# ootts/EasyHeC

Hardware: AMD Instinct MI355X
Metric: mask-render fwd+bwd frames/sec, xArm7 50k-tri @1280x720x8-view (higher is better)
Workload: dtype f32; 1 GPU; xarm7_1280x720_8view; robot=xarm7 (41096 tris, 20525 verts), views_per_gpu=8, global_views=8, links=8, antialias=True, optimizer=Adam lr 3e-3 wd 5e-4, ref_sums=bound once, mask_output=False, step=HIP launch chain, parallelism=single GPU

## Files before the change

easyhec_amd/csrc/ehr_fused_core.h:

```cpp
#pragma once
#include "ehr_host.h"
#include "ehr_pose_core.h"
#include "ehr_raster_core.h"

namespace ehr {

#define EHR_FIX_SCALE 4294967296.0
__device__ __forceinline__ long long fix_of(float v) { return __double2ll_rn((double)v * EHR_FIX_SCALE); }
__device__ __forceinline__ void fix_add(long long* acc, float v, int* meta) {
    if (!(fabsf(v) < 1.0e9f)) {
        atomicOr(&meta[EHR_META_OVERFLOW], 1);
        return;
    }
    if (v != 0.f) atomicAdd((unsigned long long*)acc, (unsigned long long)fix_of(v));
}
__device__ __forceinline__ void fix_add_delta(long long* acc, float v, long long cached, int* meta) {
    if (!(fabsf(v) < 1.0e9f)) {
        atomicOr(&meta[EHR_META_OVERFLOW], 1);
        return;
    }
    const long long d = ((v != 0.f) ? fix_of(v) : 0ll) - cached;
    if (d != 0) atomicAdd((unsigned long long*)acc, (unsigned long long)d);
}
__device__ __forceinline__ float fix_get(long long q) { return (float)((double)q * (1.0 / EHR_FIX_SCALE)); }
__device__ __forceinline__ long long acc_load(const long long* p) {
    return __hip_atomic_load(p, __ATOMIC_RELAXED, __HIP_MEMORY_SCOPE_AGENT);
}

__host__ __device__ constexpr int vb_acc_stride(int L, int nls = VB_LOSS_SLOTS) { return 12 * L + nls * VB_LOSS_STRIDE; }
__host__ __device__ __forceinline__ int* vb_acc_meta(long long* acc, int B, int L) { return (int*)(acc + (size_t)B * vb_acc_stride(L)); }

struct StepTail {
    const float* K;
    const float* link_poses;
    const float* tc_jac;
    float* red;
    float* dof;
    float* m;
    float* v;
    int* step;
    float* loss_out;
    float* grad_out;
    float n, f, lr, b1, b2, eps, wd;
    int defer_adam;
};

template <bool TAIL>
__device__ __forceinline__ void finish_body(const BinGeom& g, int B, const long long* __restrict__ facc,
                                            const long long* __restrict__ vtot, float* __restrict__ loss,
                                            float* __restrict__ grad_mvp, int* __restrict__ meta, const StepTail& tail,
                                            int nls, int* __restrict__ lbox, int lstride, float* vloss ,
                                            double (*S)[17] , float* red_lds ,
                                            float (*Js)[16] ) {
    const int tid = threadIdx.x, L = g.L;
    const int acc_stride = vb_acc_stride(L, nls);
    if (lbox)
        for (int i = tid; i < 16 * B * L; i += 256) lbox[i] = (i & 2) ? INT_MIN : INT_MAX;
    AdamState st;
    if (TAIL && !tail.defer_adam) st = pose_adam_fetch(tail.dof, tail.m, tail.v, tail.step);
    auto view_loss_slow = [&](int b) {
        long long s = vtot ? vtot[b] : 0ll;
        for (int k = 0; k < nls; k++) s += acc_load(&facc[(size_t)b * acc_stride + 12 * L + k * lstride]);
        return fix_get(s);
    };
    const bool bad = __hip_atomic_load(&meta[EHR_META_OVERFLOW], __ATOMIC_RELAXED, __HIP_MEMORY_SCOPE_AGENT) != 0;
    const float nanv = __int_as_float(0x7fc00000);
    double la_mine = 0.0;
    if (nls == 32) {
        const int k = tid & 31;
        for (int base = 0; base < B; base += 32) {
            long long s4[4];
#pragma unroll
            for (int j = 0; j < 4; j++) {
                const int b = base + 8 * j + (tid >> 5);
                s4[j] = (b < B) ? acc_load(&facc[(size_t)b * acc_stride + 12 * L + k * lstride]) : 0;
            }
            if (TAIL && base == 0 && !tail.defer_adam) pose_adam_bias(st, tail.lr, tail.b1, tail.b2);
#pragma unroll
            for (int j = 0; j < 4; j++) {
                const int b = base + 8 * j + (tid >> 5);
                if (base + 8 * j >= B) break;
                long long s = s4[j];
                s += wave_xor<16>(s);
                s += wave_xor<8>(s);
                s += wave_xor<4>(s);
                s += wave_xor<2>(s);
                s += wave_xor<1>(s);
                if (k == 0 && b < B) {
                    const float lv = bad ? nanv : fix_get(s + (vtot ? vtot[b] : 0ll));
                    loss[b] = lv;
                    la_mine += (double)lv;
                }
            }
        }
    } else {
        for (int b = tid; b < B; b += 256) {
            const float lv = bad ? nanv : view_loss_slow(b);
            loss[b] = lv;
            la_mine += (double)lv;
        }
    }
    auto grad16 = [&](int bl, float* G) {
        const int b = bl / L, l = bl - b * L;
        const long long* a = facc + (size_t)b * acc_stride + 12 * l;
        long long q[12];
#pragma unroll
        for (int e = 0; e < 12; e++) q[e] = acc_load(a + e);
#pragma unroll
        for (int e = 0; e < 16; e++) {
            const int r = e >> 2, c = e & 3;
            float v = 0.f;
            if (r != 2) v = fix_get(q[4 * (r == 3 ? 2 : r) + c]);
            G[e] = bad ? nanv : v;
        }
    };
    if (!TAIL) {
        if (grad_mvp)
            for (int i = tid; i < B * L; i += 256) {
                float G[16];
                grad16(i, G);
#pragma unroll
                for (int e = 0; e < 16; e++) grad_mvp[(size_t)i * 16 + e] = G[e];
            }
        return;
    }
    pose_backward_block_t(
        [&](int i, float* G) {
            grad16(i, G);
            if (grad_mvp)
#pragma unroll
                for (int e = 0; e < 16; e++) grad_mvp[(size_t)i * 16 + e] = G[e];
        },
        [&](int) { return 0.f; }, tail.K, tail.link_poses, tail.tc_jac, B, L, g.H, g.W, tail.n, tail.f, tail.red, S, red_lds,
        &la_mine, nls == 32, Js);
    __syncthreads();
    if (!tail.defer_adam)
        pose_adam_apply(st, tail.dof, tail.m, tail.v, tail.step, red_lds, tail.lr, tail.b1, tail.b2, tail.eps, tail.wd,
                        tail.loss_out, tail.grad_out);
}


static inline BinGeom make_geom(int H, int W, int L) {
    BinGeom g;
    g.W = W;
    g.H = H;
    g.ntx = (W + EHR_TILE_W - 1) / EHR_TILE_W;
    g.nty = (H + EHR_TILE_H - 1) / EHR_TILE_H;
    g.nt = g.ntx * g.nty;
    g.L = L;
    return g;
}

struct StepHead {
    const float* dof;
    const float* K;
    const float* link_poses;
    float* tc_jac;
    int* hist_row;
    float* history;
    int history_rows;
    float n, f;
    const int* adam_step;
    int* hstate;
};


}
```

easyhec_amd/csrc/ehr_pose_core.h:

```cpp
#pragma once
#include "ehr_device.h"

namespace ehr {

template <int N>
struct Dual {
    float v;
    float d[N];
};
template <int N>
__device__ __forceinline__ Dual<N> dconst(float c) {
    Dual<N> r;
    r.v = c;
#pragma unroll
    for (int i = 0; i < N; i++) r.d[i] = 0.f;
    return r;
}
template <int N>
__device__ __forceinline__ Dual<N> operator+(const Dual<N>& a, const Dual<N>& b) {
    Dual<N> r;
    r.v = a.v + b.v;
#pragma unroll
    for (int i = 0; i < N; i++) r.d[i] = a.d[i] + b.d[i];
    return r;
}
template <int N>
__device__ __forceinline__ Dual<N> operator-(const Dual<N>& a, const Dual<N>& b) {
    Dual<N> r;
    r.v = a.v - b.v;
#pragma unroll
    for (int i = 0; i < N; i++) r.d[i] = a.d[i] - b.d[i];
    return r;
}
template <int N>
__device__ __forceinline__ Dual<N> operator*(const Dual<N>& a, const Dual<N>& b) {
    Dual<N> r;
    r.v = a.v * b.v;
#pragma unroll
    for (int i = 0; i < N; i++) r.d[i] = a.d[i] * b.v + a.v * b.d[i];
    return r;
}
template <int N>
__device__ __forceinline__ Dual<N> operator/(const Dual<N>& a, const Dual<N>& b) {
    Dual<N> r;
    float inv = 1.f / b.v;
    r.v = a.v * inv;
#pragma unroll
    for (int i = 0; i < N; i++) r.d[i] = (a.d[i] - r.v * b.d[i]) * inv;
    return r;
}
template <int N>
__device__ __forceinline__ Dual<N> dneg(const Dual<N>& a) {
    return dconst<N>(0.f) - a;
}
template <int N>
__device__ __forceinline__ Dual<N> dsqrt(const Dual<N>& a) {
    Dual<N> r;
    r.v = sqrtf(a.v);
    float k = 0.5f / r.v;
#pragma unroll
    for (int i = 0; i < N; i++) r.d[i] = a.d[i] * k;
    return r;
}
template <int N>
__device__ __forceinline__ Dual<N> dsin(const Dual<N>& a) {
    Dual<N> r;
    r.v = sinf(a.v);
    float c = cosf(a.v);
#pragma unroll
    for (int i = 0; i < N; i++) r.d[i] = a.d[i] * c;
    return r;
}
template <int N>
__device__ __forceinline__ Dual<N> dcos(const Dual<N>& a) {
    Dual<N> r;
    r.v = cosf(a.v);
    float s = -sinf(a.v);
#pragma unroll
    for (int i = 0; i < N; i++) r.d[i] = a.d[i] * s;
    return r;
}
template <int N>
__device__ __forceinline__ Dual<N> dclamp_min(const Dual<N>& a, float eps) {
    return (a.v >= eps) ? a : dconst<N>(eps);
}

typedef Dual<6> D6;

template <int N>
__device__ void se3_exp_dual(const float* dof, float eps, Dual<N> T[16], int which = 0) {
    Dual<N> x[6];
#pragma unroll
    for (int i = 0; i < 6; i++) {
        x[i] = dconst<N>(dof[i]);
        if (N == 6) x[i].d[i % N] = 1.f;
        else if (i == which) x[i].d[0] = 1.f;
    }
    const Dual<N> u0 = x[0], u1 = x[1], u2 = x[2], w0 = x[3], w1 = x[4], w2 = x[5];
    Dual<N> nrms = w0 * w0 + w1 * w1 + w2 * w2;
    Dual<N> th = dsqrt(dclamp_min(nrms, eps));
    Dual<N> one = dconst<N>(1.f), zero = dconst<N>(0.f);
    Dual<N> inv = one / th;
    Dual<N> fac1 = inv * dsin(th);
    Dual<N> fac2 = inv * inv * (one - dcos(th));
    Dual<N> K[9] = {zero, dneg(w2), w1, w2, zero, dneg(w0), dneg(w1), w0, zero};
    Dual<N> K2[9];
    for (int r = 0; r < 3; r++)
        for (int c = 0; c < 3; c++) K2[3 * r + c] = K[3 * r] * K[c] + K[3 * r + 1] * K[3 + c] + K[3 * r + 2] * K[6 + c];
    Dual<N> fv1 = (one - dcos(th)) / (th * th);
    Dual<N> fv2 = (th - dsin(th)) / (th * th * th);
    Dual<N> u[3] = {u0, u1, u2};
    for (int r = 0; r < 3; r++) {
        Dual<N> t = zero;
        for (int c = 0; c < 3; c++) {
            Dual<N> I = dconst<N>(r == c ? 1.f : 0.f);
            T[4 * r + c] = fac1 * K[3 * r + c] + fac2 * K2[3 * r + c] + I;
            Dual<N> V = I + K[3 * r + c] * fv1 + K2[3 * r + c] * fv2;
            t = t + V * u[c];
        }
        T[4 * r + 3] = t;
    }
    T[12] = zero;
    T[13] = zero;
    T[14] = zero;
    T[15] = one;
}

__device__ __forceinline__ void mat4_mul(const float* A, const float* B, float* C) {
    for (int r = 0; r < 4; r++)
        for (int c = 0; c < 4; c++) {
            float s = A[4 * r] * B[c];
            s = fmaf(A[4 * r + 1], B[4 + c], s);
            s = fmaf(A[4 * r + 2], B[8 + c], s);
            s = fmaf(A[4 * r + 3], B[12 + c], s);
            C[4 * r + c] = s;
        }
}

__device__ __forceinline__ void projection(const float* K, int H, int W, float n, float f, float* P) {
    float fu = K[0], fv = K[4], cu = K[2], cv = K[5];
    for (int i = 0; i < 16; i++) P[i] = 0.f;
    P[0] = 2.f * fu / (float)W;
    P[2] = -2.f * cu / (float)W + 1.f;
    P[5] = 2.f * fv / (float)H;
    P[6] = 2.f * cv / (float)H - 1.f;
    P[10] = -(f + n) / (f - n);
    P[11] = -2.f * f * n / (f - n);
    P[14] = -1.f;
}


__device__ __forceinline__ void mvp_from_pose(const float* Tc, const float* P, const float* lp, float* C) {
    float A[16];
    mat4_mul(Tc, lp, A);
    for (int c = 0; c < 4; c++) {
        A[4 + c] = -A[4 + c];
        A[8 + c] = -A[8 + c];
    }
    mat4_mul(P, A, C);
}

__device__ __forceinline__ double wave_sum_f64(double v) {
    v += wave_xor<32>(v);
    v += wave_xor<16>(v);
    v += wave_xor<8>(v);
    v += wave_xor<4>(v);
    v += wave_xor<2>(v);
    v += wave_xor<1>(v);
    return v;
}
template <class GetG, class GetLoss>
__device__ __forceinline__ void pose_backward_block_t(GetG get_g, GetLoss get_loss, const float* __restrict__ K,
                                                      const float* __restrict__ link_poses,
                                                      const float* __restrict__ tc_jac, int B, int L, int H, int W,
                                                      float n, float f, float* __restrict__ red, double (*S)[17],
                                                      float* red_lds, const double* la_pre,
                                                      bool la_lanes_0_32, float (*Js_lds)[16]) {
    float (*const Js)[16] = Js_lds;
    if (threadIdx.x < 96) Js[threadIdx.x >> 4][threadIdx.x & 15] = tc_jac[16 + threadIdx.x];
    float P[16];
    projection(K, H, W, n, f, P);
    for (int r = 0; r < 4; r++) {
        P[4 * r + 1] = -P[4 * r + 1];
        P[4 * r + 2] = -P[4 * r + 2];
    }
    const int r = threadIdx.x & 3;
    double acc[4] = {0.0, 0.0, 0.0, 0.0};
    double la = 0.0;
    for (int i = threadIdx.x >> 2; i < B * L; i += blockDim.x >> 2) {
        float lp[16];
#pragma unroll
        for (int k = 0; k < 16; k++) lp[k] = link_poses[(size_t)i * 16 + k];
        float G[16];
        get_g(i, G);
        float M[4];
        for (int c = 0; c < 4; c++) {
            float s = 0.f;
            for (int k = 0; k < 4; k++) s = fmaf(P[4 * k + r], G[4 * k + c], s);
            M[c] = s;
        }
        for (int c = 0; c < 4; c++) {
            float s = 0.f;
            for (int k = 0; k < 4; k++) s = fmaf(M[k], lp[4 * c + k], s);
            acc[c] += (double)s;
        }
    }
    if (la_pre)
        la = *la_pre;
    else
        for (int i = threadIdx.x; i < B; i += blockDim.x) la += (double)get_loss(i);
    const int lane = threadIdx.x & 63, wave = threadIdx.x >> 6;
    {
        const bool b32 = lane & 32, b16 = lane & 16;
        const double a0 = (b32 ? acc[2] : acc[0]) + wave_xor<32>(b32 ? acc[0] : acc[2]);
        const double a1 = (b32 ? acc[3] : acc[1]) + wave_xor<32>(b32 ? acc[1] : acc[3]);
        double v = (b16 ? a1 : a0) + wave_xor<16>(b16 ? a0 : a1);
        v += wave_xor<8>(v);
        v += wave_xor<4>(v);
        if ((lane & 12) == 0) S[wave][4 * (lane & 3) + 2 * (b32 ? 1 : 0) + (b16 ? 1 : 0)] = v;
    }
    {
        const double s = la_lanes_0_32 ? la + wave_xor<32>(la) : wave_sum_f64(la);
        if (lane == 0) S[wave][16] = s;
    }
    __syncthreads();
    if (threadIdx.x < 8) {
        float rr;
        if (threadIdx.x < 6) {
            double g = 0.0;
            for (int k = 0; k < 16; k++)
                g += (((S[0][k] + S[1][k]) + S[2][k]) + S[3][k]) * (double)Js[threadIdx.x][k];
            rr = (float)g;
        } else {
            rr = (threadIdx.x == 6) ? (float)(((S[0][16] + S[1][16]) + S[2][16]) + S[3][16]) : (float)B;
        }
        red[threadIdx.x] = rr;
        if (red_lds) red_lds[threadIdx.x] = rr;
    }
}

__device__ __forceinline__ void pose_backward_block(const float* __restrict__ grad_mvp, const float* __restrict__ loss,
                                                    const float* __restrict__ K, const float* __restrict__ link_poses,
                                                    const float* __restrict__ tc_jac, int B, int L, int H, int W,
                                                    float n, float f, float* __restrict__ red, double (*S)[17]) {
    __shared__ float Js[6][16];
    pose_backward_block_t(
        [&](int i, float* G) {
            for (int k = 0; k < 16; k++) G[k] = grad_mvp[(size_t)i * 16 + k];
        },
        [&](int b) { return loss[b]; }, K, link_poses, tc_jac, B, L, H, W, n, f, red, S, nullptr, nullptr, false, Js);
}

struct AdamState {
    float p, m, v;
    int t;
    float step_size, rsq_bc2;
    bool has_bias;
};
__device__ __forceinline__ void pose_adam_bias(AdamState& st, float lr, float b1, float b2) {
    const float bc1 = 1.f - powf(b1, (float)st.t);
    const float bc2 = 1.f - powf(b2, (float)st.t);
    st.step_size = lr / bc1;
    st.rsq_bc2 = sqrtf(bc2);
    st.has_bias = true;
}
__device__ __forceinline__ AdamState pose_adam_fetch(const float* dof, const float* m, const float* v, const int* step) {
    AdamState st;
    st.p = st.m = st.v = 0.f;
    st.step_size = st.rsq_bc2 = 0.f;
    st.has_bias = false;
    st.t = step[0] + 1;
    if (threadIdx.x < 6) {
        st.p = dof[threadIdx.x];
        st.m = m[threadIdx.x];
        st.v = v[threadIdx.x];
    }
    return st;
}
__device__ __forceinline__ void pose_adam_apply(const AdamState& st, float* __restrict__ dof, float* __restrict__ m,
                                                float* __restrict__ v, int* __restrict__ step, const float* red, float lr,
                                                float b1, float b2, float eps, float wd, float* __restrict__ loss_out,
                                                float* __restrict__ grad_out) {
    const int i = threadIdx.x;
    const int t = st.t;
    const float nfr = red[7];
    bool ok = true;
#pragma unroll
    for (int k = 0; k < 8; k++) ok = ok && (fabsf(red[k]) < 3.0e38f);
    if (i < 6 && ok) {
        float g = red[i] / nfr;
        if (grad_out) grad_out[i] = g;
        float p = st.p;
        g = g + wd * p;
        float mi = b1 * st.m + (1.f - b1) * g;
        float vi = b2 * st.v + (1.f - b2) * g * g;
        m[i] = mi;
        v[i] = vi;
        float step_size, rsq_bc2;
        if (st.has_bias) {
            step_size = st.step_size;
            rsq_bc2 = st.rsq_bc2;
        } else {
            const float bc1 = 1.f - powf(b1, (float)t);
            const float bc2 = 1.f - powf(b2, (float)t);
            step_size = lr / bc1;
            rsq_bc2 = sqrtf(bc2);
        }
        float denom = sqrtf(vi) / rsq_bc2 + eps;
        dof[i] = p - step_size * (mi / denom);
    }
    if (i < 6 && !ok && grad_out) grad_out[i] = __int_as_float(0x7fc00000);
    if (i == 6 && loss_out) loss_out[0] = ok ? red[6] / nfr : __int_as_float(0x7fc00000);
    __syncthreads();
    if (i == 0 && ok) step[0] = t;
}
__device__ __forceinline__ void pose_adam_block(float* __restrict__ dof, float* __restrict__ m, float* __restrict__ v,
                                                int* __restrict__ step, const float* __restrict__ red, float lr,
                                                float b1, float b2, float eps, float wd, float* __restrict__ loss_out,
                                                float* __restrict__ grad_out) {
    const AdamState st = pose_adam_fetch(dof, m, v, step);
    pose_adam_apply(st, dof, m, v, step, red, lr, b1, b2, eps, wd, loss_out, grad_out);
}

}
```

easyhec_amd/csrc/ehr_vbuf.hip:

```cpp
#include <stdlib.h>
#include <string.h>

#include <algorithm>
#include <utility>
#include <vector>

#include "ehr_fused_core.h"

namespace ehr {

constexpr int VB_RW = EHR_TILE_W + 2;
constexpr int VB_RH = EHR_TILE_H + 2;
constexpr int VB_RN = VB_RW * VB_RH;
constexpr int VB_WORDS = (VB_RN + 63) / 64;
constexpr int VB_LBOX_STRIDE = 16;
constexpr int VB_HEAVY_T_DEFAULT = 3000;
constexpr int VB_HEAVY_CAP = 4096;
constexpr int VB_MED_CAP = 2048;
constexpr int VB_MED_T_DEFAULT = 1500;
constexpr int VB_PRIO_LONG = 3;
constexpr int VB_PRIO_HEAVY = 2;
constexpr int VB_JOB_ITEMS = 64;
constexpr int VB_SPILL_BLOCK = 2048;
constexpr u64 VB_EMPTY = ~0ull;
constexpr int VB_VERTEX_GRID = 5;
constexpr int VB_JOB_GRID = 4;
constexpr int VB_COMPOSITE_GRID = 6;
constexpr int VB_SCORE_COUNT_GRID = 4;
constexpr int VB_SLOW_GRID = 32;
constexpr bool VB_XCD_SPLIT = true;
constexpr int VB_FAST_EXTENT = 8192;

constexpr int VB_XCDS = 8;
constexpr int VB_XCD_BITS = __builtin_ctz(VB_XCDS);
static_assert(VB_XCDS == 1 << VB_XCD_BITS, "a workgroup finds its XCD with a mask and a shift");
__host__ __device__ constexpr int vb_xcd_share(int n) { return (n + VB_XCDS - 1) >> VB_XCD_BITS; }
__host__ __device__ constexpr int vb_xcd_round_up(int n) { return (n + VB_XCDS - 1) & ~(VB_XCDS - 1); }

enum VbLine {
    VB_LINE_JOB_CURSOR = 0,
    VB_LINE_COMP_TICKET = VB_LINE_JOB_CURSOR + VB_XCDS,
    VB_LINE_TOP_TICKET = VB_LINE_COMP_TICKET + VB_XCDS,
    VB_LINE_SLOW_COUNT,
    VB_LINES
};
__host__ __device__ __forceinline__ int* vb_line(int* meta, int k) {
    return (int*)((((uintptr_t)(meta + EHR_META_INTS)) + 127) & ~(uintptr_t)127) + 32 * k;
}
constexpr size_t VB_META_BYTES = EHR_META_INTS * sizeof(int) + (VB_LINES + 1) * 128;

#define VB_WAVE_SYNC() asm volatile("s_waitcnt lgkmcnt(0)" ::: "memory")

struct VbItem {
    int packed;
    int v1, v2;
    float alpha;
};

struct VbCarve {
    uintptr_t at;
    template <class T>
    T* take(size_t n, size_t align = alignof(T)) {
        at = (at + align - 1) & ~(uintptr_t)(align - 1);
        T* const p = (T*)at;
        at += n * sizeof(T);
        return p;
    }
};

struct VbSlots {
    float* jval;
    VbItem* jitems;
    u64* jcov;
    int* jn;
    int* jspill;
    unsigned* jid;
    int* jdesc;
    int* jbase;
    unsigned* jutile;
    int4* slow_list;
    int jcap;
};
constexpr size_t VB_SLOT_BYTES = 256 * sizeof(float) + VB_JOB_ITEMS * sizeof(VbItem) + VB_WORDS * sizeof(u64) + 2 * sizeof(int) +
                                 VB_RN * sizeof(unsigned) + sizeof(int) + sizeof(int4);
static_assert(VB_SLOT_BYTES == 1024 + 1024 + 48 + 8 + 1360 + 4 + 16, "job slot: 3484 bytes");
static VbSlots vb_slots(void* base, size_t jcap, size_t units, size_t* bytes = nullptr) {
    VbCarve c{(uintptr_t)base};
    VbSlots s;
    s.jval = c.take<float>(jcap * 256);
    s.jitems = c.take<VbItem>(jcap * VB_JOB_ITEMS);
    s.jcov = c.take<u64>(jcap * VB_WORDS);
    s.jn = c.take<int>(jcap);
    s.jspill = c.take<int>(jcap);
    s.jid = c.take<unsigned>(jcap * VB_RN);
    s.jdesc = c.take<int>(jcap);
    s.jbase = c.take<int>(units + 1);
    s.jutile = c.take<unsigned>(units);
    s.slow_list = c.take<int4>(jcap, 16);
    s.jcap = (int)jcap;
    if (bytes) *bytes = c.at - (uintptr_t)base;
    return s;
}

constexpr bool vb_interior(int i) {
    return (i % VB_RW) >= 1 && (i % VB_RW) <= EHR_TILE_W && (i / VB_RW) >= 1 && (i / VB_RW) <= EHR_TILE_H;
}
constexpr u64 vb_word_h(int k) {
    u64 w = 0;
    for (int j = 0; j < 64; j++) {
        const int i = 64 * k + j;
        if (i + 1 < VB_RN && (i % VB_RW) != VB_RW - 1 && (vb_interior(i) || vb_interior(i + 1))) w |= 1ull << j;
    }
    return w;
}
constexpr u64 vb_word_v(int k) {
    u64 w = 0;
    for (int j = 0; j < 64; j++) {
        const int i = 64 * k + j;
        if (i + VB_RW < VB_RN && (vb_interior(i) || vb_interior(i + VB_RW))) w |= 1ull << j;
    }
    return w;
}

template <int S>
__device__ __forceinline__ void vb_shr(const u64 in[VB_WORDS], u64 out[VB_WORDS]) {
#pragma unroll
    for (int k = 0; k < VB_WORDS; k++) out[k] = (in[k] >> S) | (k + 1 < VB_WORDS ? in[k + 1] << (64 - S) : 0ull);
}

__device__ __forceinline__ int vb_readlane(int v, int lane) { return __builtin_amdgcn_readlane(v, lane); }
__device__ __forceinline__ float vb_readlane(float v, int lane) {
    return __int_as_float(__builtin_amdgcn_readlane(__float_as_int(v), lane));
}
__device__ __forceinline__ float4 vb_readlane(const float4& v, int lane) {
    return make_float4(vb_readlane(v.x, lane), vb_readlane(v.y, lane), vb_readlane(v.z, lane), vb_readlane(v.w, lane));
}
__device__ __forceinline__ int vb_mbcnt(u64 m) {
    return __builtin_amdgcn_mbcnt_hi((unsigned)(m >> 32), __builtin_amdgcn_mbcnt_lo((unsigned)m, 0u));
}


struct VbHeavy {
    int* gen;
    int* list;
    int* mlist;
    int* stamp;
    int mcap;
    int heavy_base;
    int heavy_max;
};

static VbHeavy vb_heavy(void* base, size_t nstamp, size_t* bytes = nullptr) {
    VbCarve c{(uintptr_t)base};
    VbHeavy hv = {};
    hv.gen = c.take<int>(8);
    hv.list = c.take<int>(2 * VB_HEAVY_CAP);
    hv.mlist = c.take<int>(2 * VB_MED_CAP);
    hv.stamp = c.take<int>(nstamp);
    if (bytes) *bytes = c.at - (uintptr_t)base;
    return hv;
}

__device__ __forceinline__ int vb_hint_pack(int u, int tx, int ty) { return tx | (ty << 10) | (u << 22); }
__device__ __forceinline__ int vb_hint_dense(int id, int nt, int ntx) {
    return (int)((unsigned)id >> 22) * nt + ((id >> 10) & 4095) * ntx + (id & 1023);
}
static_assert(VB_MAX_UNITS <= 1024, "vb_hint_pack");
struct VbClusters {
    const int32_t* ctri;
    const int32_t* clink;
    const int32_t* coff;
    const float* laabb;
    const float4* cvert;
    int NC;
};

__device__ __forceinline__ uint2 vb_pack_box(int x0, int y0, int x1, int y1) {
    return make_uint2((unsigned)x0 | ((unsigned)y0 << 16), (unsigned)x1 | ((unsigned)y1 << 16));
}
#define VB_BOX_EMPTY make_uint2(0xffffffffu, 0u)

struct VbEdges {
    int e0, e1, e2, sx0, sx1, sx2, sy0, sy1, sy2;
};
__device__ __forceinline__ VbEdges vb_edges(int X0, int Y0, int X1, int Y1, int X2, int Y2, int bx0, int by0, int W,
                                            int H) {
    VbEdges r;
    const int ox = 16 * bx0 + 8 - 8 * W, oy = 16 * by0 + 8 - 8 * H;
    X0 -= ox; X1 -= ox; X2 -= ox;
    Y0 -= oy; Y1 -= oy; Y2 -= oy;
    {
        const int dX = X1 - X0, dY = Y1 - Y0;
        r.e0 = __mul24(dX, 0 - Y0) - __mul24(dY, 0 - X0) - (((dY < 0) || (dY == 0 && dX < 0)) ? 0 : 1);
        r.sx0 = -16 * dY;
        r.sy0 = 16 * dX;
    }
// ... 1849 lines not shown
        if (lane < VB_RH) S.cov[lane] = 0ull;
        if (COVER && lane == 0) S.bad = 0;
        VB_WAVE_SYNC();
        int nsurv = 0, dln = 0;
        const int drawn = vb_job_raster<false, COVER, LAZY>(A, S, S.key, S.cov, b, l, rg, rx0, ry0, 0, 1, nsurv, dln);
        if (COVER) {
            if (drawn >= 0 && dln > 0)
                vb_flush<true, LAZY>(S, S.key, S.cov, dln, VbLazy{pverts, pmvp + ((size_t)b * L + l) * 16, LAZY ? nullptr : posc + (size_t)b * V}, PRM(si.cvidx) + (size_t)lcoff[l] * 64, W, H, rx0, ry0);
            VB_WAVE_SYNC();
            if (drawn < 0 || S.bad) {
                if (lane == 0) PRM(rq.sl.jn)[0] = 1;
                continue;
            }
            if (drawn > 0) {
                VB_WAVE_SYNC();
                if (lane < 4) {
                    const u64 w = ((S.cov[2 * lane + 1] >> 1) & 0xffffffffull) | (((S.cov[2 * lane + 2] >> 1) & 0xffffffffull) << 32);
                    if (w) atomicOr((unsigned long long*)&PRM(rq.sl.jcov)[((((size_t)(b / PRM(rq.sl.jcap)) * gnt + (size_t)ty * gntx + tx) * PRM(rq.sl.jcap) + (b % PRM(rq.sl.jcap))) * 4 + lane)], w);
                }
            }
            continue;
        }
        if (drawn < 0) {
            if (lane == 0) vb_put_aside(PRM(rq.sl.slow_list), PRM(rq.meta), PRM(rq.sl.jn), PRM(rq.sl.jdesc), job, u, tx, ty);
            continue;
        }
        if (dln > 0) vb_flush<false, LAZY>(S, S.key, S.cov, dln, VbLazy{pverts, pmvp + ((size_t)b * L + l) * 16, LAZY ? nullptr : posc + (size_t)b * V}, PRM(si.cvidx) + (size_t)lcoff[l] * 64, W, H, rx0, ry0);
        if (lane == 0) {
            if (nsurv >= heavy_t)
                remember_heavy(hint_id);
            else if (nsurv >= med_t)
                remember_long(hint_id);
        }
        if (drawn == 0) {
            if (lane == 0) {
                PRM(rq.sl.jn)[slot] = -1;
                PRM(rq.sl.jdesc)[slot] = -1;
            }
            continue;
        }
        vb_resolve_from_lds<LAZY>(vb_prm_copy(&PRM(rq)), S, S.key, S.cov, slot, b, l, rx0, ry0);
    }
}
#undef PRM

__global__ void __launch_bounds__(256)
vb_slow_kernel(const int* __restrict__ meta, VbJobArgs A) {
    const int n = *vb_line(const_cast<int*>(meta), VB_LINE_SLOW_COUNT);
    if (n == 0) return;
    __shared__ VbWaveLds lds_all[4];
    const int wave = threadIdx.x >> 6;
    for (int i = blockIdx.x * 4 + wave; i < n; i += gridDim.x * 4) {
        const int4 e = A.sl.slow_list[i];
        if (A.posc)
            vb_job_slow<false>(A, lds_all[wave], e.x, e.y, e.z, e.w);
        else
            vb_job_slow<true>(A, lds_all[wave], e.x, e.y, e.z, e.w);
    }
}

__global__ void __launch_bounds__(256)
vb_resolve_kernel(VbResolveArgs Q) {
    __shared__ VbResolveLds lds_all[4];
    const int tid = threadIdx.x, lane = tid & 63, wave = tid >> 6;
    VbResolveLds& S = lds_all[wave];
    const int L = Q.L;
    const int n = *vb_line(Q.meta, VB_LINE_SLOW_COUNT);
    for (int it = (int)blockIdx.x * 4 + wave; it < n; it += (int)gridDim.x * 4) {
        const int job = Q.sl.slow_list[it].x;
        if (job >= Q.sl.jcap) continue;
        const size_t slot = (size_t)job;
        unsigned idw[VB_WORDS];
        {
            const unsigned* const src = Q.sl.jid + slot * VB_RN;
#pragma unroll
            for (int k = 0; k < VB_WORDS; k++) {
                const unsigned i = 64u * k + lane;
                idw[k] = (i < (unsigned)VB_RN) ? src[i] : 0xffffffffu;
            }
        }
        const u64 mycw = (lane < VB_WORDS) ? Q.sl.jcov[slot * VB_WORDS + lane] : 0ull;
        const int de = Q.sl.jdesc[job];
        if (de < 0) continue;
        const int u = de & 511, tx = (de >> 9) & 1023, ty = (de >> 19) & 4095;
        const int b = u / L;
        const int rx0 = tx * EHR_TILE_W - 1, ry0 = ty * EHR_TILE_H - 1;
        u64 C[VB_WORDS];
#pragma unroll
        for (int k = 0; k < VB_WORDS; k++) {
            const unsigned lo = (unsigned)__builtin_amdgcn_readlane((int)(unsigned)mycw, k);
            const unsigned hi = (unsigned)__builtin_amdgcn_readlane((int)(unsigned)(mycw >> 32), k);
            C[k] = ((u64)hi << 32) | lo;
        }
        VB_WAVE_SYNC();
#pragma unroll
        for (int k = 0; k < VB_WORDS; k++) {
            const unsigned i = 64u * k + lane;
            if (i < (unsigned)VB_RN)
                S.ids[i] = (idw[k] != 0xffffffffu) ? idw[k] : (((C[k] >> lane) & 1ull) ? VB_ID_COVERED : 0xffffffffu);
        }
        if (Q.posc)
            vb_resolve_job<false>(Q, S.ids, S.pairA, S.hits, C, slot, b, u - b * L, rx0, ry0);
        else
            vb_resolve_job<true>(Q, S.ids, S.pairA, S.hits, C, slot, b, u - b * L, rx0, ry0);
    }
}

__global__ void __launch_bounds__(256)
vb_refsum_kernel(BinGeom g, int B, const float* __restrict__ ref, int vec_ok, long long* __restrict__ tsum,
                 long long* __restrict__ vtot, int* __restrict__ flag) {
    const int lane = threadIdx.x & 63, wave = threadIdx.x >> 6;
    const int gw = blockIdx.x * 4 + wave;
    if (gw >= B * g.nt) return;
    const int W = g.W, H = g.H;
    const int b = gw / g.nt, tile = gw - b * g.nt;
    const int tx = tile % g.ntx, ty = tile / g.ntx;
    const int r = lane >> 3, c4 = (lane & 7) * 4;
    const int ix = tx * EHR_TILE_W + c4, iy = ty * EHR_TILE_H + r;
    const bool row_in = iy < H;
    const size_t im = ((size_t)b * H + (H - 1 - (row_in ? iy : 0))) * W + ix;
    float rf[4] = {0.f, 0.f, 0.f, 0.f};
    bool pin[4];
#pragma unroll
    for (int j = 0; j < 4; j++) pin[j] = row_in && (ix + j) < W;
    if (vec_ok) {
        if (pin[0]) {
            const float4 r4 = *reinterpret_cast<const float4*>(ref + im);
            rf[0] = r4.x; rf[1] = r4.y; rf[2] = r4.z; rf[3] = r4.w;
        }
    } else {
#pragma unroll
        for (int j = 0; j < 4; j++)
            if (pin[j]) rf[j] = ref[im + j];
    }
    float e2 = 0.f;
#pragma unroll
    for (int j = 0; j < 4; j++)
        if (pin[j]) {
            const float e = 0.f - rf[j];
            e2 += e * e;
        }
    const float s = wave_sum(e2);
    if (lane == 0) {
        long long q = 0;
        if (!(fabsf(s) < 1.0e9f))
            atomicOr(flag, 1);
        else if (s != 0.f)
            q = fix_of(s);
        tsum[gw] = q;
        if (q != 0) atomicAdd((unsigned long long*)&vtot[b], (unsigned long long)q);
    }
}

template <bool TAIL, bool FILL>
__global__ void __launch_bounds__(256, FILL ? 5 : 6)
vb_composite_kernel(VbCompArgs C, StepTail tail) {
    __shared__ float gpix_all[4][EHR_TILE_W * EHR_TILE_H];
    extern __shared__ int s_dyn[];
    const int tid = threadIdx.x, lane = tid & 63, wave = tid >> 6;
    float* const gpix = gpix_all[wave];
    const int U = C.B * C.g.L;
    int* const s_jbase = s_dyn;
    unsigned* const s_utile = reinterpret_cast<unsigned*>(s_dyn + U + 1);
    const bool sparse = C.tsum != nullptr;
    for (int i = tid; i <= U; i += 256) s_jbase[i] = C.sl.jbase[i];
    for (int i = tid; i < U; i += 256) s_utile[i] = C.sl.jutile[i];
    if (C.do_finish && C.lbox_all)
        for (int i = (int)blockIdx.x * 256 + tid; i < VB_LBOX_STRIDE * C.B_all * C.g.L; i += (int)gridDim.x * 256)
            C.lbox_all[i] = (i & 2) ? INT_MIN : INT_MAX;
    __syncthreads();
    const int nwg = gridDim.x, xcd = blockIdx.x & (VB_XCDS - 1);
    vb_composite_items<FILL>(C, s_jbase, s_utile, gpix, xcd, (int)(blockIdx.x >> VB_XCD_BITS) * 4 + wave, (nwg >> VB_XCD_BITS) * 4, nwg);
    if (!C.do_finish) return;
    asm volatile("s_waitcnt vmcnt(0)" ::: "memory");
    __syncthreads();
    __shared__ int s_last;
    if (tid == 0) {
        int last = 0;
        const int per = nwg >> VB_XCD_BITS;
        int* const xcd_ticket = vb_line(C.meta, VB_LINE_COMP_TICKET + xcd);
        int* const top_ticket = vb_line(C.meta, VB_LINE_TOP_TICKET);
        if (atomicAdd(xcd_ticket, 1) == per - 1) last = atomicAdd(top_ticket, 1) == VB_XCDS - 1;
        s_last = last;
    }
    __syncthreads();
    if (!s_last) return;
    if (C.ref_flag && tid == 0 && C.ref_flag[0]) atomicOr(&C.meta[EHR_META_OVERFLOW], 1);
    __syncthreads();
    __shared__ double S[4][17];
    __shared__ float red_lds[8];
    __shared__ float Js[6][16];
    finish_body<TAIL>(C.g, C.B_all, C.facc_all, sparse ? C.vtot_all : nullptr, C.loss, C.grad_mvp, C.meta, tail, C.nls, nullptr,
                      VB_LOSS_STRIDE, gpix_all[0], S, red_lds, Js);
}

__global__ void __launch_bounds__(256)
vb_hash_kernel(const unsigned* __restrict__ a, size_t na, const unsigned* __restrict__ b, size_t nb, const unsigned* __restrict__ c,
               size_t nc, unsigned long long* __restrict__ out) {
    unsigned long long h = 0;
    const size_t n = na + nb + nc;
    for (size_t i = (size_t)blockIdx.x * 256 + threadIdx.x; i < n; i += (size_t)gridDim.x * 256) {
        const unsigned w = i < na ? a[i] : (i < na + nb ? b[i - na] : c[i - na - nb]);
        unsigned long long x = (unsigned long long)w + 0x9e3779b97f4a7c15ull * ((unsigned long long)i + 1ull);
        x ^= x >> 33;
        x *= 0xff51afd7ed558ccdull;
        x ^= x >> 33;
        x *= 0xc4ceb9fe1a85ec53ull;
        x ^= x >> 33;
        h += x;
    }
#pragma unroll
    for (int o = 32; o > 0; o >>= 1) h += __shfl_xor(h, o, 64);
    if ((threadIdx.x & 63) == 0) atomicAdd(out, h);
}

__global__ void __launch_bounds__(256)
vb_score_count_kernel(BinGeom g, int nq, int S, const u64* __restrict__ tcov, unsigned long long* __restrict__ sacc,
                      unsigned char* __restrict__ count_img, int* __restrict__ lbox, int nlbox,
                      unsigned long long* __restrict__ prev_sacc, long long* __restrict__ prev_score, int prev_nq) {
    const int lane = threadIdx.x & 63, wave = threadIdx.x >> 6;
    for (int i = blockIdx.x * 256 + threadIdx.x; i < nlbox; i += gridDim.x * 256) lbox[i] = (i & 2) ? INT_MIN : INT_MAX;
    if (blockIdx.x == 0)
        for (int i = threadIdx.x; i < prev_nq; i += 256) {
            prev_score[i] = (long long)prev_sacc[16 * i];
            prev_sacc[16 * i] = 0ull;
        }
    const int r = lane >> 3, c4 = (lane & 7) * 4;
    const int sh = (r & 1) * 32 + c4;
    for (int item = blockIdx.x * 4 + wave; item < nq * g.nt; item += gridDim.x * 4) {
    const int q = item / g.nt, tile = item - q * g.nt;
    int c[4] = {0, 0, 0, 0};
    for (int s0 = 0; s0 < S; s0 += 16) {
        const int ls = s0 + (lane >> 2);
        const u64 mine = (ls < S) ? tcov[(((size_t)q * g.nt + tile) * S + ls) * 4 + (lane & 3)] : 0ull;
        if (__ballot(mine != 0ull) == 0) continue;

        const int ns = min(16, S - s0);
        for (int k = 0; k < ns; k++) {
            const int src = 4 * k + (r >> 1);
            const unsigned lo = (unsigned)__shfl((int)(unsigned)mine, src, 64), hi = (unsigned)__shfl((int)(unsigned)(mine >> 32), src, 64);
            const unsigned bits = (unsigned)(((((u64)hi) << 32) | lo) >> sh) & 15u;
#pragma unroll
            for (int j = 0; j < 4; j++) c[j] += (bits >> j) & 1u;
        }
    }
    int v = 0;
#pragma unroll
    for (int j = 0; j < 4; j++) v += c[j] * (S - c[j]);
#pragma unroll
    for (int o = 32; o > 0; o >>= 1) v += __shfl_xor(v, o, 64);
    if (lane == 0 && v) atomicAdd(&sacc[16 * q], (unsigned long long)v);
    if (count_img) {
        const int tx = tile % g.ntx, ty = tile / g.ntx;
        const int ix = tx * EHR_TILE_W + c4, iy = ty * EHR_TILE_H + r;
        if (iy < g.H)
#pragma unroll
            for (int j = 0; j < 4; j++)
                if (ix + j < g.W && c[j]) count_img[((size_t)q * g.H + (g.H - 1 - iy)) * g.W + ix + j] = (unsigned char)c[j];
    }
    }
}

__global__ void vb_pad_kernel(const int32_t* __restrict__ a, int T, int4* __restrict__ out) {
    const int t = blockIdx.x * blockDim.x + threadIdx.x;
    if (t < T) out[t] = make_int4(a[3 * t], a[3 * t + 1], a[3 * t + 2], 0);
}

}
using namespace ehr;


static void vb_kd_order(const float* cen, int* idx, int n) {
    if (n <= 64) return;
    float lo[3] = {3.4e38f, 3.4e38f, 3.4e38f}, hi[3] = {-3.4e38f, -3.4e38f, -3.4e38f};
    for (int i = 0; i < n; i++)
        for (int k = 0; k < 3; k++) {
            const float c = cen[3 * (size_t)idx[i] + k];
            lo[k] = std::min(lo[k], c);
            hi[k] = std::max(hi[k], c);
        }
    int ax = 0;
    if (hi[1] - lo[1] > hi[ax] - lo[ax]) ax = 1;
    if (hi[2] - lo[2] > hi[ax] - lo[ax]) ax = 2;
    const int half = std::min(std::max(((n / 2 + 63) / 64) * 64, 64), n - 1);
    std::nth_element(idx, idx + half, idx + n, [&](int a, int b) {
        const float ca = cen[3 * (size_t)a + ax], cb = cen[3 * (size_t)b + ax];
        return ca < cb || (ca == cb && a < b);
    });
    vb_kd_order(cen, idx, half);
    vb_kd_order(cen, idx + half, n - half);
}

static int vb_build_clusters(Scratch& out, int& nc_out, int L, int V, int T, const float* verts, const int32_t* tris,
                             const int32_t* tri_link, const int32_t* vert_link = nullptr, bool* mixed = nullptr) {
    std::vector<float> hv((size_t)3 * std::max(V, 1));
    std::vector<int32_t> ht((size_t)3 * std::max(T, 1)), hl((size_t)std::max(T, 1));
    if (V > 0) EHR_HIP(hipMemcpy(hv.data(), verts, (size_t)3 * V * sizeof(float), hipMemcpyDeviceToHost));
    if (T > 0) {
        EHR_HIP(hipMemcpy(ht.data(), tris, (size_t)3 * T * sizeof(int32_t), hipMemcpyDeviceToHost));
        if (tri_link) {
            EHR_HIP(hipMemcpy(hl.data(), tri_link, (size_t)T * sizeof(int32_t), hipMemcpyDeviceToHost));
        } else {
            std::vector<int32_t> vl((size_t)std::max(V, 1), 0);
            if (V > 0) EHR_HIP(hipMemcpy(vl.data(), vert_link, (size_t)V * sizeof(int32_t), hipMemcpyDeviceToHost));
            int prev = 0;
            for (int t = 0; t < T; t++) {
                int lk[3];
                for (int j = 0; j < 3; j++) {
                    const int v = ht[3 * (size_t)t + j];
                    lk[j] = ((unsigned)v < (unsigned)V) ? vl[v] : -1;
                }
                if (lk[0] != lk[1] || lk[0] != lk[2] || (unsigned)lk[0] >= (unsigned)L || lk[0] < prev) {
                    *mixed = true;
                    return EHR_OK;
                }
                prev = lk[0];
                hl[t] = lk[0];
            }
        }
    }
    std::vector<int32_t> ctri, clink, coff((size_t)L + 1, 0);
    std::vector<float> aabb((size_t)6 * L);
    for (int l = 0; l < L; l++)
        for (int k = 0; k < 3; k++) {
            aabb[6 * (size_t)l + k] = 3.4e38f;
            aabb[6 * (size_t)l + 3 + k] = -3.4e38f;
        }
    int t = 0;
    for (int l = 0; l < L; l++) {
        coff[l] = (int32_t)clink.size();
        const int t0 = t;
        while (t < T && hl[t] == l) t++;
        if (t < T && hl[t] < l) return fail(EHR_ERR_INVALID, "ehr_fused_plan: tri_link must be sorted by link");
        const int n = t - t0;
        if (n == 0) continue;
        std::vector<float> cen((size_t)3 * n);
        float lo[3] = {3.4e38f, 3.4e38f, 3.4e38f}, hi[3] = {-3.4e38f, -3.4e38f, -3.4e38f};
        for (int i = 0; i < n; i++)
            for (int k = 0; k < 3; k++) {
                float c = 0.f;
                for (int j = 0; j < 3; j++) {
                    const int v = ht[3 * (size_t)(t0 + i) + j];
                    const float x = ((unsigned)v < (unsigned)V) ? hv[3 * (size_t)v + k] : 0.f;
                    c += x;
                    if ((unsigned)v < (unsigned)V) {
                        aabb[6 * (size_t)l + k] = std::min(aabb[6 * (size_t)l + k], x);
// ... 450 lines not shown
```

Before: 113,700 frames/s.

## Replace last-block ticket finish with designated finisher polling per-XCD arrivals

The composite kernel used to elect the last-arriving block through two levels of atomic tickets, and that block then ran the loss, pose-backward and Adam finish. Now one fixed block is the finisher. Only blocks that actually had work increment a per-XCD arrival counter, and the finisher prefetches the Adam state, projection columns, Jacobian and link poses into LDS while it polls the counters. This overlaps the finish setup latency with the tail of the composite work and cuts atomics from idle blocks. It risks a spin-wait deadlock if the finisher is scheduled before the producing blocks, which is handled by a poll cap that sets an overflow flag, and it relies on the arrival-count formula matching the real work distribution.

```diff
diff --git a/easyhec_amd/csrc/ehr_fused_core.h b/easyhec_amd/csrc/ehr_fused_core.h
--- a/easyhec_amd/csrc/ehr_fused_core.h
+++ b/easyhec_amd/csrc/ehr_fused_core.h
@@ -45,19 +45,34 @@
     int defer_adam;
 };
 
+struct FinishPre {
+    AdamState st;
+    PoseBwdPre pb;
+    long long vt;
+};
+
 template <bool TAIL>
-__device__ __forceinline__ void finish_body(const BinGeom& g, int B, const long long* __restrict__ facc,
-                                            const long long* __restrict__ vtot, float* __restrict__ loss,
-                                            float* __restrict__ grad_mvp, int* __restrict__ meta, const StepTail& tail,
-                                            int nls, int* __restrict__ lbox, int lstride, float* vloss ,
-                                            double (*S)[17] , float* red_lds ,
-                                            float (*Js)[16] ) {
+__device__ __forceinline__ void finish_prefetch(FinishPre& pre, const BinGeom& g, int B, const long long* __restrict__ vtot,
+                                                const StepTail& tail, int nls, float (*Js)[16] ,
+                                                float* lp_lds ) {
+    const int tid = threadIdx.x;
+    if (TAIL && !tail.defer_adam) pre.st = pose_adam_fetch(tail.dof, tail.m, tail.v, tail.step);
+    pre.vt = (nls == 32 && vtot && (tid & 31) == 0 && (tid >> 5) < B) ? vtot[tid >> 5] : 0ll;
+    if (TAIL) {
+        pose_backward_prefetch(pre.pb, tail.K, tail.link_poses, tail.tc_jac, B, g.L, g.H, g.W, tail.n, tail.f, Js, lp_lds);
+        if (!tail.defer_adam) pose_adam_bias(pre.st, tail.lr, tail.b1, tail.b2);
+    }
+}
+
+template <bool TAIL>
+__device__ __forceinline__ void finish_reduce(const FinishPre& pre, const BinGeom& g, int B, const long long* __restrict__ facc,
+                                              const long long* __restrict__ vtot, float* __restrict__ loss,
+                                              float* __restrict__ grad_mvp, int* __restrict__ meta, const StepTail& tail,
+                                              int nls, int lstride, double (*S)[17] ,
+                                              float* red_lds , float (*Js)[16] ,
+                                              const float* lp_lds ) {
     const int tid = threadIdx.x, L = g.L;
     const int acc_stride = vb_acc_stride(L, nls);
-    if (lbox)
-        for (int i = tid; i < 16 * B * L; i += 256) lbox[i] = (i & 2) ? INT_MIN : INT_MAX;
-    AdamState st;
-    if (TAIL && !tail.defer_adam) st = pose_adam_fetch(tail.dof, tail.m, tail.v, tail.step);
     auto view_loss_slow = [&](int b) {
         long long s = vtot ? vtot[b] : 0ll;
         for (int k = 0; k < nls; k++) s += acc_load(&facc[(size_t)b * acc_stride + 12 * L + k * lstride]);
@@ -75,7 +90,6 @@
                 const int b = base + 8 * j + (tid >> 5);
                 s4[j] = (b < B) ? acc_load(&facc[(size_t)b * acc_stride + 12 * L + k * lstride]) : 0;
             }
-            if (TAIL && base == 0 && !tail.defer_adam) pose_adam_bias(st, tail.lr, tail.b1, tail.b2);
 #pragma unroll
             for (int j = 0; j < 4; j++) {
                 const int b = base + 8 * j + (tid >> 5);
@@ -87,7 +101,7 @@
                 s += wave_xor<2>(s);
                 s += wave_xor<1>(s);
                 if (k == 0 && b < B) {
-                    const float lv = bad ? nanv : fix_get(s + (vtot ? vtot[b] : 0ll));
+                    const float lv = bad ? nanv : fix_get(s + (vtot ? (base + j == 0 ? pre.vt : vtot[b]) : 0ll));
                     loss[b] = lv;
                     la_mine += (double)lv;
                 }
@@ -124,18 +138,17 @@
             }
         return;
     }
-    pose_backward_block_t(
+    pose_backward_reduce_t(
         [&](int i, float* G) {
             grad16(i, G);
             if (grad_mvp)
 #pragma unroll
                 for (int e = 0; e < 16; e++) grad_mvp[(size_t)i * 16 + e] = G[e];
         },
-        [&](int) { return 0.f; }, tail.K, tail.link_poses, tail.tc_jac, B, L, g.H, g.W, tail.n, tail.f, tail.red, S, red_lds,
-        &la_mine, nls == 32, Js);
+        [&](int) { return 0.f; }, pre.pb, tail.link_poses, B, L, tail.red, S, red_lds, &la_mine, nls == 32, Js, lp_lds);
     __syncthreads();
     if (!tail.defer_adam)
-        pose_adam_apply(st, tail.dof, tail.m, tail.v, tail.step, red_lds, tail.lr, tail.b1, tail.b2, tail.eps, tail.wd,
+        pose_adam_apply(pre.st, tail.dof, tail.m, tail.v, tail.step, red_lds, tail.lr, tail.b1, tail.b2, tail.eps, tail.wd,
                         tail.loss_out, tail.grad_out);
 }
 
diff --git a/easyhec_amd/csrc/ehr_pose_core.h b/easyhec_amd/csrc/ehr_pose_core.h
--- a/easyhec_amd/csrc/ehr_pose_core.h
+++ b/easyhec_amd/csrc/ehr_pose_core.h
@@ -169,34 +169,48 @@
     v += wave_xor<1>(v);
     return v;
 }
-template <class GetG, class GetLoss>
-__device__ __forceinline__ void pose_backward_block_t(GetG get_g, GetLoss get_loss, const float* __restrict__ K,
-                                                      const float* __restrict__ link_poses,
-                                                      const float* __restrict__ tc_jac, int B, int L, int H, int W,
-                                                      float n, float f, float* __restrict__ red, double (*S)[17],
-                                                      float* red_lds, const double* la_pre,
-                                                      bool la_lanes_0_32, float (*Js_lds)[16]) {
-    float (*const Js)[16] = Js_lds;
-    if (threadIdx.x < 96) Js[threadIdx.x >> 4][threadIdx.x & 15] = tc_jac[16 + threadIdx.x];
+struct PoseBwdPre {
+    float Pc[4];
+};
+__device__ __forceinline__ void pose_backward_prefetch(PoseBwdPre& pre, const float* __restrict__ K,
+                                                       const float* __restrict__ link_poses,
+                                                       const float* __restrict__ tc_jac, int B, int L, int H, int W,
+                                                       float n, float f, float (*Js_lds)[16], float* lp_lds) {
+    if (threadIdx.x < 96) Js_lds[threadIdx.x >> 4][threadIdx.x & 15] = tc_jac[16 + threadIdx.x];
     float P[16];
     projection(K, H, W, n, f, P);
     for (int r = 0; r < 4; r++) {
         P[4 * r + 1] = -P[4 * r + 1];
         P[4 * r + 2] = -P[4 * r + 2];
     }
-    const int r = threadIdx.x & 3;
+    for (int k = 0; k < 4; k++) pre.Pc[k] = P[4 * k + (threadIdx.x & 3)];
+    if (lp_lds && (int)threadIdx.x < 4 * min(B * L, 64))
+        reinterpret_cast<float4*>(lp_lds)[threadIdx.x] = reinterpret_cast<const float4*>(link_poses)[threadIdx.x];
+}
+template <class GetG, class GetLoss>
+__device__ __forceinline__ void pose_backward_reduce_t(GetG get_g, GetLoss get_loss, const PoseBwdPre& pre,
+                                                       const float* __restrict__ link_poses, int B, int L,
+                                                       float* __restrict__ red, double (*S)[17], float* red_lds,
+                                                       const double* la_pre, bool la_lanes_0_32, float (*Js_lds)[16],
+                                                       const float* lp_lds) {
+    float (*const Js)[16] = Js_lds;
     double acc[4] = {0.0, 0.0, 0.0, 0.0};
     double la = 0.0;
     for (int i = threadIdx.x >> 2; i < B * L; i += blockDim.x >> 2) {
         float lp[16];
-#pragma unroll
-        for (int k = 0; k < 16; k++) lp[k] = link_poses[(size_t)i * 16 + k];
+        if (lp_lds && i < 64) {
+#pragma unroll
+            for (int k = 0; k < 16; k++) lp[k] = lp_lds[i * 16 + k];
+        } else {
+#pragma unroll
+            for (int k = 0; k < 16; k++) lp[k] = link_poses[(size_t)i * 16 + k];
+        }
         float G[16];
         get_g(i, G);
         float M[4];
         for (int c = 0; c < 4; c++) {
             float s = 0.f;
-            for (int k = 0; k < 4; k++) s = fmaf(P[4 * k + r], G[4 * k + c], s);
+            for (int k = 0; k < 4; k++) s = fmaf(pre.Pc[k], G[4 * k + c], s);
             M[c] = s;
         }
         for (int c = 0; c < 4; c++) {
@@ -237,6 +251,17 @@
         red[threadIdx.x] = rr;
         if (red_lds) red_lds[threadIdx.x] = rr;
     }
+}
+template <class GetG, class GetLoss>
+__device__ __forceinline__ void pose_backward_block_t(GetG get_g, GetLoss get_loss, const float* __restrict__ K,
+                                                      const float* __restrict__ link_poses,
+                                                      const float* __restrict__ tc_jac, int B, int L, int H, int W,
+                                                      float n, float f, float* __restrict__ red, double (*S)[17],
+                                                      float* red_lds, const double* la_pre,
+                                                      bool la_lanes_0_32, float (*Js_lds)[16]) {
+    PoseBwdPre pre;
+    pose_backward_prefetch(pre, K, link_poses, tc_jac, B, L, H, W, n, f, Js_lds, nullptr);
+    pose_backward_reduce_t(get_g, get_loss, pre, link_poses, B, L, red, S, red_lds, la_pre, la_lanes_0_32, Js_lds, nullptr);
 }
 
 __device__ __forceinline__ void pose_backward_block(const float* __restrict__ grad_mvp, const float* __restrict__ loss,
diff --git a/easyhec_amd/csrc/ehr_vbuf.hip b/easyhec_amd/csrc/ehr_vbuf.hip
--- a/easyhec_amd/csrc/ehr_vbuf.hip
+++ b/easyhec_amd/csrc/ehr_vbuf.hip
@@ -39,9 +39,8 @@
 
 enum VbLine {
     VB_LINE_JOB_CURSOR = 0,
-    VB_LINE_COMP_TICKET = VB_LINE_JOB_CURSOR + VB_XCDS,
-    VB_LINE_TOP_TICKET = VB_LINE_COMP_TICKET + VB_XCDS,
-    VB_LINE_SLOW_COUNT,
+    VB_LINE_COMP_ARRIVE = VB_LINE_JOB_CURSOR + VB_XCDS,
+    VB_LINE_SLOW_COUNT = VB_LINE_COMP_ARRIVE + VB_XCDS,
     VB_LINES
 };
 __host__ __device__ __forceinline__ int* vb_line(int* meta, int k) {
@@ -2197,6 +2196,28 @@
     }
 }
 
+struct VbCompParams {
+    VbCompArgs C;
+    StepTail tail;
+};
+typedef const VbCompParams __attribute__((address_space(4)))* VbCompParamsPtr;
+__device__ __forceinline__ VbCompParamsPtr vb_comp_params() {
+    VbCompParamsPtr p = (VbCompParamsPtr)__builtin_amdgcn_kernarg_segment_ptr();
+    asm volatile("" : "+s"(p));
+    return p;
+}
+
+constexpr int VB_FINISH_POLLS = 1 << 21;
+__device__ __forceinline__ int vb_comp_arrivals(int xcd, int per, int nitems, int nfill, int nlbox) {
+    const int share = vb_xcd_share(nitems);
+    const int mine = max(0, min(share, nitems - xcd * share));
+    int n = (mine + 3) >> 2;
+    const int fwg = (nfill + 3) >> 2, lwg = (nlbox + 255) >> 8;
+    n = max(n, fwg > xcd ? vb_xcd_share(fwg - xcd) : 0);
+    n = max(n, lwg > xcd ? vb_xcd_share(lwg - xcd) : 0);
+    return min(n, per);
+}
+
 template <bool TAIL, bool FILL>
 __global__ void __launch_bounds__(256, FILL ? 5 : 6)
 vb_composite_kernel(VbCompArgs C, StepTail tail) {
@@ -2216,27 +2237,49 @@
     __syncthreads();
     const int nwg = gridDim.x, xcd = blockIdx.x & (VB_XCDS - 1);
     vb_composite_items<FILL>(C, s_jbase, s_utile, gpix, xcd, (int)(blockIdx.x >> VB_XCD_BITS) * 4 + wave, (nwg >> VB_XCD_BITS) * 4, nwg);
-    if (!C.do_finish) return;
-    asm volatile("s_waitcnt vmcnt(0)" ::: "memory");
-    __syncthreads();
-    __shared__ int s_last;
-    if (tid == 0) {
-        int last = 0;
-        const int per = nwg >> VB_XCD_BITS;
-        int* const xcd_ticket = vb_line(C.meta, VB_LINE_COMP_TICKET + xcd);
-        int* const top_ticket = vb_line(C.meta, VB_LINE_TOP_TICKET);
-        if (atomicAdd(xcd_ticket, 1) == per - 1) last = atomicAdd(top_ticket, 1) == VB_XCDS - 1;
-        s_last = last;
-    }
-    __syncthreads();
-    if (!s_last) return;
-    if (C.ref_flag && tid == 0 && C.ref_flag[0]) atomicOr(&C.meta[EHR_META_OVERFLOW], 1);
-    __syncthreads();
+    if (!vb_comp_params()->C.do_finish) return;
+    const VbCompParamsPtr Q = vb_comp_params();
+    const int per = nwg >> VB_XCD_BITS;
+    const int nitems = sparse ? min(s_jbase[U], Q->C.sl.jcap) : Q->C.B * Q->C.g.nt;
+    const int nfill = FILL ? Q->C.B * Q->C.g.nt : 0, nlbox = Q->C.lbox_all ? VB_LBOX_STRIDE * Q->C.B_all * Q->C.g.L : 0;
+    const int kblk = (int)(blockIdx.x >> VB_XCD_BITS);
+    const bool finisher = (int)blockIdx.x == nwg - VB_XCDS;
+    const bool arrives = kblk < vb_comp_arrivals(xcd, per, nitems, nfill, nlbox);
+    if (!finisher) {
+        if (!arrives) return;
+        asm volatile("s_waitcnt vmcnt(0)" ::: "memory");
+        __syncthreads();
+        if (tid == 0)
+            (void)__hip_atomic_fetch_add(vb_line(Q->C.meta, VB_LINE_COMP_ARRIVE + xcd), 1, __ATOMIC_RELAXED, __HIP_MEMORY_SCOPE_AGENT);
+        return;
+    }
     __shared__ double S[4][17];
     __shared__ float red_lds[8];
     __shared__ float Js[6][16];
-    finish_body<TAIL>(C.g, C.B_all, C.facc_all, sparse ? C.vtot_all : nullptr, C.loss, C.grad_mvp, C.meta, tail, C.nls, nullptr,
-                      VB_LOSS_STRIDE, gpix_all[0], S, red_lds, Js);
+    const long long* const vtot = sparse ? Q->C.vtot_all : nullptr;
+    const BinGeom g = ((const VbCompParams*)Q)->C.g;
+    const StepTail tl = ((const VbCompParams*)Q)->tail;
+    FinishPre pre;
+    __syncthreads();
+    finish_prefetch<TAIL>(pre, g, Q->C.B_all, vtot, tl, Q->C.nls, Js, gpix_all[0]);
+    if (Q->C.ref_flag && tid == 0 && Q->C.ref_flag[0]) atomicOr(&Q->C.meta[EHR_META_OVERFLOW], 1);
+    if (wave == 0) {
+        int* const ctr = vb_line(Q->C.meta, VB_LINE_COMP_ARRIVE + (lane & (VB_XCDS - 1)));
+        const int want = vb_comp_arrivals(lane & (VB_XCDS - 1), per, nitems, nfill, nlbox) - (((lane & (VB_XCDS - 1)) == 0 && arrives) ? 1 : 0);
+        bool done = false;
+        for (int polls = 0; polls < VB_FINISH_POLLS; polls++) {
+            const int have = (lane < VB_XCDS) ? __hip_atomic_load(ctr, __ATOMIC_RELAXED, __HIP_MEMORY_SCOPE_AGENT) : want;
+            done = __ballot(have < want) == 0;
+            if (done) break;
+            __builtin_amdgcn_s_sleep(2);
+        }
+        if (lane < VB_XCDS) __hip_atomic_store(ctr, 0, __ATOMIC_RELAXED, __HIP_MEMORY_SCOPE_AGENT);
+        if (!done && lane == 0) atomicOr(&Q->C.meta[EHR_META_OVERFLOW], 1);
+    }
+    asm volatile("s_waitcnt vmcnt(0)" ::: "memory");
+    __syncthreads();
+    __builtin_amdgcn_fence(__ATOMIC_ACQUIRE, "agent");
+    finish_reduce<TAIL>(pre, g, Q->C.B_all, Q->C.facc_all, vtot, Q->C.loss, Q->C.grad_mvp, Q->C.meta, tl, Q->C.nls, VB_LOSS_STRIDE, S, red_lds, Js, gpix_all[0]);
 }
 
 __global__ void __launch_bounds__(256)
```

After: 117,600 frames/s (median of 6 runs). +3.5%, better.
